# yukara-ikemiya/world-class

Measured on AMD Instinct MI355X. Metric: analysis+synthesis frames/sec (whole node), 48 kHz 5 ms hop, higher is better.
Workload: dtype f64; 1 GPU; 64 synthetic 48 kHz 10 s utterances per GPU (8 distinct, tiled), 5 ms hop, Harvest->CheapTrick->D4C->Synthesis, inputs resident in HBM when the clock starts (`value`; SURVEY.md section 8(d)'s headline with H2D of x and D2H of all outputs inside the clock is `value_with_transfers`); utterances_per_gpu=64, frames_per_gpu=128064, fs=48000, fft_size=2048, parallelism=utterance-sharded x1 (shard.partition), final RCCL all-gather of F0 + checksums

## Files before the change

### world_class_amd/csrc/wc_d4c.hip

```cpp
#include <cmath>
#include <cstdio>
#include <cstdlib>
#include <cstring>
#include <type_traits>
#include <vector>

#include "wc_device.hpp"
#include "wc_internal.hpp"
#include "wc_frames.hpp"
#include "wc_wavefft.hpp"
#include "wc_hostcopy.hpp"

namespace wc {

constexpr double kSafe = 0.000000000001;
constexpr int kMaxBands = 5;

struct D4cArgs {
	const double *x;
	const UttDesc *utts;
	int n_utt;
	const double *tpos, *f0;
	const unsigned long long *rng_off;
	const uint32_t *rng_table;
	unsigned long long rng_base;
	const double2 *tw;
	double *ap;
	double *ap0;
	double *sgd;
	double *coarse;
	uint32_t *cnt;
	const double *nuttall;
	long long total_frames;
	int fs, fft_size_out, n_ap, window_length;
	int select64;
	double threshold;
	long long sgd_stride;
	int *long_list, *long_cnt;
	const int *uidx;
	int rare_only;
	int *rare_list;
	int *lt_list;
	unsigned int *band_tails;
};

template <int N, int T>
__device__ __forceinline__ int d4c_windowed(const double *__restrict__ x, int x_len, int fs, double f0, double pos,
											int type, double ratio, const uint32_t *__restrict__ rng,
											unsigned long long roff, double (&wave)[N / T], double *red, int tid) {
	constexpr int EPT = N / T;
	asm volatile("" : "+v"(tid));
	const int hw = mround(ratio * fs / f0 / 2.0);
	const int wl = 2 * hw + 1;
	const int origin = mround(pos * fs + 0.001);
	const double c1 = 2.0 / ratio / fs;
	double cs0, sn0, csd, snd;
	sincospi(f0 * (c1 * (tid - hw)), &sn0, &cs0);
	sincospi(f0 * (c1 * T), &snd, &csd);
	snd = uniform_d(snd);
	csd = uniform_d(csd);
	auto win = [&](double c) { return type == 1 ? fma(0.5, c, 0.5) : fma(c, fma(0.16, c, 0.5), 0.34); };
	double s1 = 0.0, s2 = 0.0;
	{
		double c = cs0, sn = sn0;
#pragma unroll
		for (int e = 0; e < EPT; ++e) {
			const int i = tid + e * T;
			const bool in = i < wl;
			const double w = in ? win(c) : 0.0;
			const int si = clampi(origin + i - hw, 0, x_len - 1);
			const double noise = randn_at(rng, roff + (in ? i : 0)) * kSafe;
			wave[e] = in ? fma(x[si], w, noise) : 0.0;
			s1 += wave[e];
			s2 += w;
			const double cn = fma(c, csd, -(sn * snd));
			sn = fma(sn, csd, c * snd);
			c = cn;
		}
	}
	block_sum2<T>(s1, s2, red, tid);
	const double wc = uniform_d(s1 / s2);
	{
		double c = cs0, sn = sn0;
#pragma unroll
		for (int e = 0; e < EPT; ++e) {
			const int i = tid + e * T;
			wave[e] = fma(-(i < wl ? win(c) : 0.0), wc, wave[e]);
			const double cn = fma(c, csd, -(sn * snd));
			sn = fma(sn, csd, c * snd);
			c = cn;
		}
// ... 526 lines not shown
		acc = __shfl(acc, first, 64);
		d = __shfl(d, first, 64);
		in_bucket = __shfl(cnt, first, 64);
		need -= acc;
		pre |= ((unsigned long long)d) << shift;
		if (in_bucket == 1u) break;
	}
	double low = 0.0, eq = 0.0, tot = 0.0;
#pragma unroll
	for (int e = 0; e < KEYS; ++e) {
		if (e < nkeys) {
			const double pw = key[e];
			const unsigned long long hb = ((unsigned long long)__double_as_longlong(pw)) >> shift;
			tot += pw;
			low += (hb < (pre >> shift)) ? pw : 0.0;
			eq += (hb == (pre >> shift)) ? pw : 0.0;
		}
	}
	block_sum3<T>(low, eq, tot, red3, tid);
	if (tid == 0) {
		const double thr = (in_bucket == 1u) ? eq : __longlong_as_double((long long)pre);
		const double part = low + (double)need * thr;
		const double cv = 10 * log10(part / tot);
		a.coarse[g * kMaxBands + bnd] = fmin(0.0, cv + (f0 - 100) / 50.0);
	}
}

__global__ __launch_bounds__(256) void d4c_rows_kernel(D4cArgs a) {
	const long long g = blockIdx.x;
	const double f0v = a.f0[g];
	if (f0v == 0.0 || a.ap0[g] <= a.threshold) return;
	const int n_ap = a.n_ap, fs = a.fs;
	const int bins_out = a.fft_size_out / 2 + 1;
	const double *__restrict__ co = a.coarse + g * kMaxBands;
	double *__restrict__ row = a.ap + g * (long long)bins_out;
	const int na = n_ap + 2;
	auto val = [&](int q) { return q == 0 ? -60.0 : (q == na - 1 ? -kSafe : co[q - 1]); };
	for (int k = threadIdx.x; k < bins_out; k += 256) {
		double f = (double)k * fs / a.fft_size_out;
		int c = 1;
		while (c < na && f >= ((c == na - 1) ? fs / 2.0 : c * 3000.0)) ++c;
		c = min(c, na - 1);
		double x0 = (c - 1) * 3000.0;
		double x1 = (c == na - 1) ? fs / 2.0 : c * 3000.0;
		double s = (f - x0) / (x1 - x0);
		double v = val(c - 1) + s * (val(c) - val(c - 1));
		row[k] = exp(v * 0.11512925464970228);
	}
}


constexpr long long kD4Row = 4160;
constexpr int kD4Lds = 2304;

template <int SLOTS>
__device__ __forceinline__ int d4c2_windowed(int type, const double *__restrict__ x, int x_last, int fs, double f0, double pos, double ratio,
											 const uint32_t *__restrict__ rng, int odd, bool weighted, double (&re)[16],
											 double (&im)[16], double &sumsq, int lane) {
	WC_FRESH(lane);
	const int hw = __builtin_amdgcn_readfirstlane(mround(ratio * fs / f0 / 2.0));
	const int wl = 2 * hw + 1;
	const int base = __builtin_amdgcn_readfirstlane(mround(pos * fs + 0.001)) - hw;
	const double c1 = 2.0 / ratio / fs;
	double ce0, se0, co0, so0, cd, sd;
	wf_sincospi(f0 * (c1 * (2 * lane - hw)), se0, ce0);
	wf_sincospi(f0 * (c1 * (2 * lane + 1 - hw)), so0, co0);
	wf_sincospi(f0 * (c1 * 128.0), sd, cd);
	sd = uniform_d(sd);
	cd = uniform_d(cd);
	const double a0 = type == 1 ? 0.5 : 0.34, a2 = type == 1 ? 0.0 : 0.16;
	auto win = [&](double c) { return fma(c, fma(a2, c, 0.5), a0); };
	auto walk = [&](auto loads_c, auto &&body) {
		constexpr int LOADS = decltype(loads_c)::value;
		double ce = ce0, se = se0, co = co0, so = so0;
#pragma unroll
		for (int qg = 0; qg < SLOTS; qg += 4) {
			if (qg * 128 >= wl) break;
			double xs[8];
			uint32_t ns[8];
			const bool ld = LOADS == 1 || (LOADS == 2 && qg >= 16);
			if (ld) {
#pragma unroll
				for (int k = 0; k < 8; ++k) {
					const int i = 2 * lane + 128 * (qg + (k >> 1)) + (k & 1);
					xs[k] = x[clampi(base + i, 0, x_last)];
					ns[k] = rng[i < wl ? i : 0];
				}
				WF_SCHED_FENCE();
			}
#pragma unroll
			for (int k = 0; k < 4; ++k) {
				const int q = qg + k, i0 = 2 * lane + 128 * q;
				const double We = (i0 < wl) ? win(ce) : 0.0, Wo = (i0 + 1 < wl) ? win(co) : 0.0;
				const double ve = (ld && i0 < wl) ? fma(xs[2 * k], We, (ns[2 * k] / 268435456.0 - 6.0) * kSafe) : 0.0;
				const double vo = (ld && i0 + 1 < wl) ? fma(xs[2 * k + 1], Wo, (ns[2 * k + 1] / 268435456.0 - 6.0) * kSafe) : 0.0;
				body(q, i0, We, Wo, ve, vo);
				const double cen = fma(ce, cd, -(se * sd)), con = fma(co, cd, -(so * sd));
				se = fma(se, cd, ce * sd);
				so = fma(so, cd, co * sd);
				ce = cen;
				co = con;
			}
		}
	};
#pragma unroll
	for (int q = 0; q < 16; ++q) re[q] = im[q] = 0.0;
	double s1 = 0.0, s2 = 0.0;
	walk(std::integral_constant<int, 1>(), [&](int q, int, double We, double Wo, double ve, double vo) {
		if (q < 16) { re[q] = ve; im[q] = vo; }
		s1 += ve + vo;
		s2 += We + Wo;
	});
	s1 = wave_sum_all(s1);
	s2 = wave_sum_all(s2);
	const double wc = s1 / s2;
	sumsq = 0.0;
	walk(std::integral_constant<int, 2>(), [&](int q, int i0, double We, double Wo, double ve, double vo) {
		if (q < 16) { ve = re[q]; vo = im[q]; }
		ve = fma(-We, wc, ve);
		vo = fma(-Wo, wc, vo);
		sumsq = fma(vo, vo, fma(ve, ve, sumsq));
		if (weighted) { ve *= i0 + 1.0; vo *= i0 + 2.0; }
		if (q < 16) { re[q] = ve; im[q] = vo; }
		else if (odd) { re[q & 15] -= ve; im[q & 15] -= vo; }
		else { re[q & 15] += ve; im[q & 15] += vo; }
	});
	sumsq = wave_sum_all(sumsq);
	return wl;
}
__device__ __forceinline__ int d4c2_groups(int wl) { return wl > 2048 ? 4 : (wl + 511) >> 9; }

#ifndef WC_D4C2_LT_OCC
#define WC_D4C2_LT_OCC 2
#endif
template <bool LONG>
__device__ __forceinline__ void d4c2_lovetrain_frame(const D4cArgs &a, long long g, double *L, int lane) {
	constexpr int N = 4096, M = 2048;
	const int bins_out = a.fft_size_out / 2 + 1;
	double *__restrict__ row = a.ap + g * (long long)bins_out;
	const double f0v = a.f0[g];
	const int fs = a.fs;
	const double f0c = uniform_d(fmax(f0v, 40.0));
	const bool is_long = f0v != 0.0 && 2 * mround(3.0 * fs / f0c / 2.0) + 1 > 2048;
	if (is_long != LONG) return;
	double ap0 = 0.0;
	if (f0v != 0.0) {
		const int u = a.uidx[g];
		const UttDesc ud = a.utts[u];
		const int b0 = (int)ceil(100.0 * N / fs);
		const int b1 = (int)ceil(4000.0 * N / fs);
		const int b2 = min((int)ceil(7900.0 * N / fs), M);
		double p1 = 0.0, p2 = 0.0;
		double mr[16], mi[16], unused;
		int wl = 0;
		if (!LONG) wl = d4c2_windowed<16>(2, a.x + ud.x_off, ud.x_len - 1, fs, f0c, a.tpos[g], 3.0, a.rng_table + (a.rng_off[g] - a.rng_base), 0,
										  false, mr, mi, unused, lane);
#pragma unroll 1
		for (int odd = 0; odd < 2; ++odd) {
			double re[16], im[16], nyq;
			if (LONG) {
				wl = d4c2_windowed<32>(2, a.x + ud.x_off, ud.x_len - 1, fs, f0c, a.tpos[g], 3.0, a.rng_table + (a.rng_off[g] - a.rng_base), odd,
									   false, re, im, unused, lane);
			} else {
#pragma unroll
				for (int q = 0; q < 16; ++q) { re[q] = mr[q]; im[q] = mi[q]; }
			}
			wf_r2c4096_half(re, im, nyq, d4c2_groups(wl), L, a.tw, lane, odd);
#pragma unroll
			for (int gq = 0; gq < 4; ++gq) {
				const int j = wf_j(lane, odd, gq);
#pragma unroll
				for (int q = 0; q < 4; ++q) {
					const int k = 2 * (j + 256 * q) + odd;
					const double p = fma(re[4 * gq + q], re[4 * gq + q], im[4 * gq + q] * im[4 * gq + q]);
					p2 += (k > b0 && k <= b2) ? p : 0.0;
					p1 += (k > b0 && k <= min(b1, b2)) ? p : 0.0;
				}
			}
// ... 75 lines not shown
			for (int q = 0; q < 4; ++q) L[jg[p][gq] + 512 * q + b] = s.v[p][4 * gq + q] * fs / N;
	if (lane == 0) L[M + b] = s.vM * fs / N;
	{
		const int ke = 2 * lane, ko = 2 * lane + 1;
		if (ke >= 1 && ke <= b) {
			L[b - ke] = s.v[0][0] * fs / N;
			L[M + b + ke] = s.v[0][7] * fs / N;
		}
		if (ko <= b) {
			L[b - ko] = s.v[1][0] * fs / N;
			L[M + b + ko] = s.v[1][7] * fs / N;
		}
	}
	wf_fence();
	if (NONNEG) {
		seq_cumsum_nonneg_wave<36>(L, len, lane);
	} else {
		seq_cumsum_signed_wave<36>(L, len, lane);
	}
	const double step = (double)fs / N;
	const double origin_axis = -(b - 0.5) * fs / N;
	const double rstep = 1.0 / step;
	const double rwidth = uniform_d(1.0 / width);
	auto at = [&](int k) {
		const double lo_axis = (double)k / N * fs - width / 2.0, hi_axis = lo_axis + width;
		return (wf_interp1q(origin_axis, step, rstep, L, len, hi_axis) - wf_interp1q(origin_axis, step, rstep, L, len, lo_axis)) * rwidth;
	};
#pragma unroll
	for (int p = 0; p < 2; ++p)
#pragma unroll
		for (int gq = 0; gq < 4; ++gq) {
#pragma unroll
			for (int q = 0; q < 4; ++q) s.v[p][4 * gq + q] = at(jg[p][gq] + 512 * q);
			WF_SCHED_FENCE();
		}
	s.vM = at(M);
	wf_fence();
}

#ifndef WC_D4C2_OCC
#define WC_D4C2_OCC 2
#endif
#ifndef WC_D4C2_MASTER_LDS
#define WC_D4C2_MASTER_LDS 1
#endif
#ifndef WC_D4C2_TRACE
#define WC_D4C2_TRACE 0
#endif
#if WC_D4C2_TRACE
#define D4_STAMP(i) do { if (lane == 0) reinterpret_cast<unsigned long long *>(park + 4128)[i] = __builtin_readcyclecounter(); } while (0)
#else
#define D4_STAMP(i) do { } while (0)
#endif
#ifndef WC_D4C2_BUFFER
#define WC_D4C2_BUFFER 1
#endif
#if WC_D4C2_BUFFER
typedef unsigned int d4_u2 __attribute__((ext_vector_type(2)));
struct D4Row { __amdgpu_buffer_rsrc_t r; };
__device__ __forceinline__ D4Row d4_row(double *p) {
	D4Row w;
	w.r = __builtin_amdgcn_make_buffer_rsrc(p, 0, (int)(kD4Row * 8), 0x00020000);
	return w;
}
__device__ __forceinline__ double d4_ld(const D4Row &w, int idx) {
	const d4_u2 v = __builtin_amdgcn_raw_buffer_load_b64(w.r, idx * 8, 0, 0);
	return __hiloint2double((int)v.y, (int)v.x);
}
__device__ __forceinline__ void d4_st(const D4Row &w, int idx, double d) {
	d4_u2 v;
	v.x = (unsigned)__double2loint(d);
	v.y = (unsigned)__double2hiint(d);
	__builtin_amdgcn_raw_buffer_store_b64(v, w.r, idx * 8, 0, 0);
}
#else
struct D4Row { double *p; };
__device__ __forceinline__ D4Row d4_row(double *p) { D4Row w; w.p = p; asm volatile("" : "+s"(w.p)); return w; }
__device__ __forceinline__ double d4_ld(const D4Row &w, int idx) { return w.p[idx]; }
__device__ __forceinline__ void d4_st(const D4Row &w, int idx, double d) { w.p[idx] = d; }
#endif
template <bool LONG>
__device__ __forceinline__ void d4c2_frame(const D4cArgs &a, const long long g, double *L, const int lane) {
	constexpr int M = 2048;
	const double f0v = a.f0[g];
	if (f0v == 0.0 || a.ap0[g] <= a.threshold) return;
	const int fs = a.fs;
	const double f0 = uniform_d(fmax(47.0, f0v));
	if (!d4c2_can(f0, fs)) {
		if (!LONG && lane == 0) a.rare_list[1 + atomicAdd(a.rare_list, 1)] = (int)g;
		return;
	}
	const int wl = __builtin_amdgcn_readfirstlane(2 * mround(4.0 * fs / f0 / 2.0) + 1);
	if constexpr (!LONG) {
		if (wl > 2048) {
			if (lane == 0) a.long_list[1 + atomicAdd(a.long_cnt, 1)] = (int)g;
			return;
		}
	}
	const int u = a.uidx[g];
	const UttDesc ud = a.utts[u];
	const double *__restrict__ x = a.x + ud.x_off;
	const int x_last = ud.x_len - 1;
	const double pos = uniform_d(a.tpos[g]);
	const uint32_t *__restrict__ rng = a.rng_table + (a.rng_off[g] - a.rng_base);
#ifdef WC_D4C2_PARK_ALIAS
	double *park = a.sgd + (g & 2047) * a.sgd_stride;
#else
	double *park = a.sgd + g * a.sgd_stride;
#endif
	const D4Row row = d4_row(park);
	D4_STAMP(0);

	const int ng = d4c2_groups(wl);
	double cenM = 0.0, spsM = 0.0;
	if constexpr (!LONG) {
#pragma unroll 1
		for (int job = 0; job < 3; ++job) {
			int ln = lane;
			WC_FRESH(ln);
			const double p = (job == 0) ? pos - 0.25 / f0 : (job == 1) ? pos + 0.25 / f0 : pos;
			double pw;
			{
				double mr[16], mi[16], sumsq;
				d4c2_windowed<16>(job == 2 ? 1 : 2, x, x_last, fs, f0, p, 4.0, rng + (long long)job * wl, 0, false, mr, mi, sumsq, ln);
				pw = (job == 2) ? 1.0 : 0.5 * (1.0 / sqrt(sumsq));
#pragma unroll
				for (int q = 0; q < 16; ++q) {
					if (q < 4 * ng) {
						if (WC_D4C2_MASTER_LDS && job != 2) L[kWfLds + 64 * q + ln] = mr[q] * pw;
						else d4_st(row, 2048 + 64 * q + ln, mr[q] * pw);
						d4_st(row, 3072 + 64 * q + ln, mi[q] * pw);
					}
				}
				if (job == 0) D4_STAMP(1);
			}
			auto master = [&](double (&re)[16], double (&im)[16], bool weighted) {
// ... 12 lines not shown
				if (weighted) {
#pragma unroll
					for (int q = 0; q < 16; ++q) {
						const int i0 = 2 * ln + 128 * q;
						re[q] *= i0 + 1.0;
						im[q] *= i0 + 2.0;
					}
				}
			};
#pragma unroll 1
			for (int odd = 0; odd < 2; ++odd) {
				double re[16], im[16], nyq1;
				master(re, im, false);
				wf_r2c4096_half(re, im, nyq1, ng, L, a.tw, ln, odd);
				if (job == 0 && odd == 0) D4_STAMP(2);
				if (job == 2) {
					double pwr[16];
#pragma unroll
					for (int s = 0; s < 16; ++s) pwr[s] = 0.25 * fma(re[s], re[s], im[s] * im[s]);
					if (odd == 0) {
						spsM = 0.25 * (nyq1 * nyq1);
#pragma unroll
						for (int s = 0; s < 16; ++s) L[kWfLds + 64 * s + ln] = pwr[s];
					} else {
#pragma unroll
						for (int s = 0; s < 16; ++s) {
							d4_st(row, 3072 + 64 * s + ln, pwr[s]);
							d4_st(row, 2048 + 64 * s + ln, L[kWfLds + 64 * s + ln]);
						}
					}
				} else {
					double ar[16], ai[16], nyq2;
					master(ar, ai, true);
					wf_r2c4096_half(ar, ai, nyq2, ng, L, a.tw, ln, odd);
					double acc[16];
#pragma unroll
					for (int s = 0; s < 16; ++s) acc[s] = fma(re[s], ar[s], im[s] * ai[s]);
					if (job == 1) {
						double prev[16];
#pragma unroll
						for (int s = 0; s < 16; ++s) prev[s] = d4_ld(row, 1024 * odd + 64 * s + ln);
						WF_SCHED_FENCE();
#pragma unroll
						for (int s = 0; s < 16; ++s) acc[s] += prev[s];
					}
#pragma unroll
					for (int s = 0; s < 16; ++s) d4_st(row, 1024 * odd + 64 * s + ln, acc[s]);
					if (odd == 0) cenM += nyq1 * nyq2;
					if (job == 0 && odd == 0) D4_STAMP(3);
				}
			}
			if (job == 0) D4_STAMP(4);
		}
	} else
#pragma unroll 1
	for (int odd = 0; odd < 2; ++odd) {
		double acc[16], accM = 0.0;
#pragma unroll
		for (int s = 0; s < 16; ++s) acc[s] = 0.0;
#pragma unroll 1
		for (int job = 0; job < 3; ++job) {
			int ln = lane;
			WC_FRESH(ln);
			double ar[16], ai[16], re[16], im[16], sumsq, nyq1;
			const double p = (job == 0) ? pos - 0.25 / f0 : (job == 1) ? pos + 0.25 / f0 : pos;
			d4c2_windowed<32>(job == 2 ? 1 : 2, x, x_last, fs, f0, p, 4.0, rng + (long long)job * wl, odd, false, ar, ai, sumsq, ln);
			if (odd == 0 && job == 0) D4_STAMP(1);
			const double pw = (job == 2) ? 1.0 : 0.5 * (1.0 / sqrt(sumsq));
#pragma unroll
			for (int q = 0; q < 16; ++q) {
				re[q] = ar[q] * pw;
				im[q] = ai[q] * pw;
			}
			wf_r2c4096_half(re, im, nyq1, ng, L, a.tw, lane, odd);
			if (odd == 0 && job == 0) D4_STAMP(2);
			if (job == 2) {
#pragma unroll
				for (int s = 0; s < 16; ++s) d4_st(row, 2048 + 1024 * odd + 64 * s + ln, 0.25 * fma(re[s], re[s], im[s] * im[s]));
				if (odd == 0) spsM = 0.25 * (nyq1 * nyq1);
			} else {
				double nyq2;
				if (wl > 2048) {
					d4c2_windowed<32>(2, x, x_last, fs, f0, p, 4.0, rng + (long long)job * wl, odd, true, ar, ai, sumsq, ln);
#pragma unroll
					for (int q = 0; q < 16; ++q) { ar[q] *= pw; ai[q] *= pw; }
				} else {
#pragma unroll
					for (int q = 0; q < 16; ++q) {
						const int i0 = 2 * ln + 128 * q;
						ar[q] *= pw * (i0 + 1.0);
						ai[q] *= pw * (i0 + 2.0);
					}
				}
				wf_r2c4096_half(ar, ai, nyq2, ng, L, a.tw, lane, odd);
#pragma unroll
				for (int s = 0; s < 16; ++s) acc[s] += fma(re[s], ar[s], im[s] * ai[s]);
				accM += nyq1 * nyq2;
				if (odd == 0 && job == 0) D4_STAMP(3);
			}
		}
#pragma unroll
		for (int s = 0; s < 16; ++s) d4_st(row, 1024 * odd + 64 * s + lane, acc[s]);
		if (odd == 0) cenM = accM;
		if (odd == 0) D4_STAMP(4);
	}
	D4_STAMP(5);
	D4Bins cen, sps;
#pragma unroll
	for (int p = 0; p < 2; ++p)
#pragma unroll
		for (int s = 0; s < 16; ++s) {
			cen.v[p][s] = d4_ld(row, 1024 * p + 64 * s + lane);
			sps.v[p][s] = d4_ld(row, 2048 + 1024 * p + 64 * s + lane);
		}
	cen.vM = cenM;
	sps.vM = spsM;
	D4_STAMP(6);
	d4c2_dc_correction(cen, f0, fs, L, lane);
	d4c2_dc_correction(sps, f0, fs, L, lane);
	D4_STAMP(7);
	d4c2_smooth<true>(sps, f0, fs, L, lane);
	D4_STAMP(8);
#pragma unroll
	for (int p = 0; p < 2; ++p)
#pragma unroll
		for (int s = 0; s < 16; ++s) cen.v[p][s] = cen.v[p][s] / sps.v[p][s];
	cen.vM = cen.vM / sps.vM;
#pragma unroll 1
	for (int it = 0; it < 2; ++it) {
		d4c2_smooth<false>(cen, it ? f0 : f0 / 2.0, fs, L, lane);
		if (it == 0) sps = cen;
	}
	D4_STAMP(9);
#pragma unroll
	for (int p = 0; p < 2; ++p)
#pragma unroll
		for (int gq = 0; gq < 4; ++gq) {
			const int j = 2 * wf_j(lane, p, gq) + p;
#pragma unroll
			for (int q = 0; q < 4; ++q) d4_st(row, j + 512 * q, sps.v[p][4 * gq + q] - cen.v[p][4 * gq + q]);
		}
	if (lane == 0) d4_st(row, M, sps.vM - cen.vM);
	D4_STAMP(10);
}

template <bool LONG>
__global__ __launch_bounds__(64) __attribute__((amdgpu_waves_per_eu(WC_D4C2_OCC, WC_D4C2_OCC))) void d4c2_frames_kernel(D4cArgs a) {
	__shared__ __attribute__((aligned(16))) double L[kD4Lds];
	const int lane = threadIdx.x;
	if constexpr (!LONG) {
		const long long g = xcd_frame(blockIdx.x, a.total_frames);
		if (g >= a.total_frames) return;
		d4c2_frame<false>(a, g, L, lane);
	} else {
		const int n_long = *a.long_cnt;
#pragma unroll 1
		for (int i = blockIdx.x; i < n_long; i += gridDim.x) {
			d4c2_frame<true>(a, a.long_list[1 + i], L, lane);
			wf_fence();
		}
	}
}

#ifndef WC_D4C2_BAND_OCC
#define WC_D4C2_BAND_OCC 2
#endif
#ifndef WC_D4C2_BRACKET
#define WC_D4C2_BRACKET 1
#endif
#ifndef WC_D4C2_BRACKET_FIRST
#define WC_D4C2_BRACKET_FIRST 0x1p-14
#endif
#ifndef WC_D4C2_BAND_PF
#define WC_D4C2_BAND_PF 0
#endif
template <int WAVES>
__global__ __launch_bounds__(64) __attribute__((amdgpu_waves_per_eu(WAVES == 3 ? 3 : WC_D4C2_BAND_OCC, WAVES == 3 ? 3 : WC_D4C2_BAND_OCC))) void d4c2_band_kernel(D4cArgs a) {
	constexpr int N = 4096, M = 2048;
	constexpr bool W3 = WAVES == 3;
	__shared__ __attribute__((aligned(16))) double L[kWfLds + (W3 ? kWfT2Lds : 0)];
	const double *T2 = W3 ? L + kWfLds : nullptr;
	if constexpr (W3) __builtin_assume(T2 != nullptr);
	const int lane = threadIdx.x;
	const int n_ap = a.n_ap;
	const long long blk = xcd_frame(blockIdx.x, (long long)gridDim.x);
	const long long g = blk / n_ap;
	const int bnd = (int)(blk % n_ap);
	if (g >= a.total_frames) return;
	const double f0v = a.f0[g];
	if (f0v == 0.0 || a.ap0[g] <= a.threshold) return;
	if constexpr (W3) wf_t2_to_lds(L + kWfLds, a.tw, lane);
	const double f0 = fmax(47.0, f0v);
	const int fs = a.fs;
	const int wln = a.window_length, hwl = wln / 2;
	const int boundary = mround(N * 8.0 / wln);
	const unsigned int K = (unsigned int)(M + 1 - boundary - 1);
	const int center = (int)(3000.0 * (bnd + 1) * N / fs);
	const double *__restrict__ src = a.sgd + g * a.sgd_stride + (center - hwl);
	const int ng = wln > 512 ? 2 : 1;
	double key[2][16], keyM = 0.0;
	[[maybe_unused]] double pf = 0.0;
	auto half = [&](auto parity) {
		constexpr int odd = decltype(parity)::value;
		double re[16], im[16], nyq;
		int ln = lane;
		if constexpr (W3) WC_FRESH(ln);
		{
			double sv[16], nv[16];
#pragma unroll
			for (int k = 0; k < 16; ++k) {
				const int i = min(2 * ln + 128 * (k >> 1) + (k & 1), wln - 1);
				sv[k] = src[i];
				nv[k] = a.nuttall[i];
// ... 459 lines not shown
		while (hi_h - lo_h > 1 && c_lo != K) {
			const int mid = lo_h + ((hi_h - lo_h) >> 1);
			const unsigned int c = count_hi(mid);
			if (c >= K) hi_h = mid;
			if (c <= K) { lo_h = mid; c_lo = c; }
		}
		lo = lo_h < 0 ? -1ll : (((long long)lo_h << 32) | 0xFFFFFFFFll);
		hi = min(hi, ((long long)hi_h << 32) | 0xFFFFFFFFll);
	} else {
#pragma unroll 1
		for (int tr = 0; tr < 2; ++tr) {
			const long long cand = __double_as_longlong(mx * (tr == 0 ? WC_D4C2_BRACKET_FIRST : 0x1p-40));
			const unsigned int c = count_le(cand);
			if (c <= K && cand > 0) { lo = cand; c_lo = c; break; }
			hi = cand > 0 && c >= K ? cand : hi;
		}
	}
	for (int it = 0; it < 64 && hi - lo > 1 && c_lo != K; ++it) {
		const long long mid = lo + ((hi - lo) >> 1);
		const unsigned int c = count_le(mid);
		if (c >= K) hi = mid;
		if (c <= K) { lo = mid; c_lo = c; }
		if (c == K) break;
	}
	double low = 0.0, tot = 0.0;
#pragma unroll
	for (int s = 0; s < 16; ++s) {
		tot += key[s];
		low += (__double_as_longlong(key[s]) <= lo) ? key[s] : 0.0;
	}
	if (lane == 0) {
		tot += keyM;
		low += (__double_as_longlong(keyM) <= lo) ? keyM : 0.0;
	}
	low = wave_sum_all(low);
	tot = wave_sum_all(tot);
	if (lane == 0) {
		const double part = low + (double)(K - c_lo) * __longlong_as_double(hi);
		const double cv = 10 * log10(part / tot);
		a.coarse[g * kMaxBands + bnd] = fmin(0.0, cv + (f0 - 100) / 50.0);
	}
}

}

using namespace wc;

struct wc_d4c {
	int fs, fft_size_d4c, fft_size_lt, n_ap, window_length;
	double threshold;
	bool select64 = false;
	int band_waves = 3;
	bool lt_listed = true;
	bool count_tails = false;
	bool split;
	bool wave2;
	Device *dev;
	double f0_bound = 0.0;
	DevBuf nuttall, utts, cnt, uidx, long_list, rare_list, lt_list, tails, off, endpos, endpos2, ap0, sgd, coarse, d_x, d_tpos, d_f0, d_ap;
	HostBuf h_stage, h_rows, h_x;
};

template <int N>
static void launch_lt(const D4cArgs &a, hipStream_t s) {
	long long blocks = ((a.total_frames + 7) / 8) * 8;
	constexpr int TL = (N >= 8192) ? 1024 : (N / 8 < 64 ? 64 : N / 8);
	hipLaunchKernelGGL((d4c_lovetrain_kernel<N, TL>), dim3((unsigned)blocks), dim3(TL), 0, s, a);
}
template <int N>
static void launch_main(const D4cArgs &a, hipStream_t s, bool split, int part) {
	long long blocks = ((a.total_frames + 7) / 8) * 8;
	constexpr int TF = (N >= 8192) ? 1024 : (N / 8 < 64 ? 64 : N / 8);
	if (part == 0) {
		if (!split) hipLaunchKernelGGL((d4c_frames_kernel<N, TF, false>), dim3((unsigned)blocks), dim3(TF), 0, s, a);
		else hipLaunchKernelGGL((d4c_frames_kernel<N, TF, true>), dim3((unsigned)blocks), dim3(TF), 0, s, a);
		return;
	}
	if (a.n_ap > 0) hipLaunchKernelGGL((d4c_band_kernel<N, TF>), dim3((unsigned)(blocks * a.n_ap)), dim3(TF), 0, s, a);
	hipLaunchKernelGGL(d4c_rows_kernel, dim3((unsigned)a.total_frames), dim3(256), 0, s, a);
}

int d4c_enqueue(wc_d4c *d, hipStream_t s, int n_utt, const double *d_x, const int *x_length, const double *d_tpos,
				const double *d_f0, const int *f0_length, int fft_size, double *d_ap, const uint64_t *rng_pos,
				const unsigned long long *d_start) {
	Device *dev = d->dev;
	if (fft_size < 2 || (fft_size & 1)) return fail(WC_ERR_INVALID, "d4c: fft_size must be even and positive");
	std::vector<UttDesc> utts(n_utt);
	long long xo = 0, fo = 0;
	uint64_t min_pos = ~0ull, max_end = 0;
	const uint64_t lt_max = (uint64_t)(2 * (int)(3.0 * d->fs / 40.0 / 2.0 + 1.0) + 1);
	const uint64_t main_max = 3ull * (uint64_t)(2 * (int)(4.0 * d->fs / 47.0 / 2.0 + 1.0) + 1);
	for (int u = 0; u < n_utt; ++u) {
		if (x_length[u] <= 0 || f0_length[u] < 0) return fail(WC_ERR_INVALID, "d4c: non-positive length");
		UttDesc &t = utts[u];
		t.x_off = xo; t.f_off = fo; t.y_off = 0;
		t.x_len = x_length[u]; t.f_len = f0_length[u]; t.y_len = 0; t.f_base = 0;
		t.rng_pos = rng_pos ? rng_pos[u] : 0ull;
		xo += x_length[u];
		fo += f0_length[u];
		if (t.rng_pos < min_pos) min_pos = t.rng_pos;
		uint64_t e = t.rng_pos + (lt_max + main_max) * (uint64_t)t.f_len;
		if (e > max_end) max_end = e;
	}
	const long long total = fo;
	(void)min_pos; (void)max_end;
	if (total == 0) return WC_OK;
	int rc;
	if ((rc = d->utts.reserve(sizeof(UttDesc) * n_utt))) return rc;
	if ((rc = d->cnt.reserve(sizeof(uint32_t) * total))) return rc;
	if ((rc = d->uidx.reserve(sizeof(int) * total))) return rc;
	if ((rc = d->long_list.reserve(sizeof(int) * (total + 1)))) return rc;
	if ((rc = d->rare_list.reserve(sizeof(int) * (total + 1)))) return rc;
	if ((rc = d->off.reserve(sizeof(uint64_t) * total))) return rc;
	if ((rc = d->ap0.reserve(sizeof(double) * total))) return rc;
	const bool split = d->split;
	const bool main2 = d->wave2 && split && (d->fft_size_d4c == 4096 || d->fft_size_d4c == 2048) && d->window_length <= 1023;
	const long long row2 = d->fft_size_d4c == 4096 ? kD4Row : kD4Row1;
	if (split) {
		if ((rc = d->sgd.reserve(sizeof(double) * (size_t)total * (main2 ? (size_t)row2 : (size_t)(d->fft_size_d4c / 2 + 1))))) return rc;
		if ((rc = d->coarse.reserve(sizeof(double) * (size_t)total * kMaxBands))) return rc;
	}
	if ((rc = d->endpos.reserve(sizeof(uint64_t) * n_utt))) return rc;
	if ((rc = d->endpos2.reserve(sizeof(uint64_t) * n_utt))) return rc;
	if ((rc = d->h_stage.reserve(sizeof(UttDesc) * n_utt + sizeof(uint64_t) * n_utt))) return rc;
	std::memcpy(d->h_stage.p, utts.data(), sizeof(UttDesc) * n_utt);
	WC_HIP(hipMemcpyAsync(d->utts.p, d->h_stage.p, sizeof(UttDesc) * n_utt, hipMemcpyHostToDevice, s));
	if ((rc = d->h_stage.mark(s))) return rc;
	const unsigned grid1 = (unsigned)((total + 255) / 256);
	const bool lt_listed = d->lt_listed && d->wave2 && d->fft_size_lt == 4096;
	if (lt_listed) {
		if ((rc = d->lt_list.reserve(sizeof(int) * (total + 1)))) return rc;
		WC_HIP(hipMemsetAsync(d->lt_list.p, 0, sizeof(int), s));
	}
	if (d->count_tails) {
		if ((rc = d->tails.reserve(sizeof(unsigned int)))) return rc;
		WC_HIP(hipMemsetAsync(d->tails.p, 0, sizeof(unsigned int), s));
	}
	hipLaunchKernelGGL(d4c_lt_count_kernel, dim3(grid1), dim3(256), 0, s, d_f0, total, d->fs, d->cnt.as<uint32_t>(), d->utts.as<UttDesc>(), n_utt,
					   d->uidx.as<int>(), d->long_list.as<int>(), d->rare_list.as<int>(), lt_listed ? d->lt_list.as<int>() : nullptr);
	hipLaunchKernelGGL(utt_scan_kernel, dim3(n_utt), dim3(256), 0, s, d->cnt.as<uint32_t>(), d->utts.as<UttDesc>(),
					   d_start, d->off.as<unsigned long long>(), d->endpos.as<unsigned long long>());
	D4cArgs a;
	a.x = d_x; a.utts = d->utts.as<UttDesc>(); a.n_utt = n_utt; a.tpos = d_tpos; a.f0 = d_f0;
	a.rng_off = d->off.as<unsigned long long>(); a.rng_table = dev->rng_table.as<uint32_t>(); a.rng_base = dev->rng_base;
	a.tw = dev->twiddle; a.ap = d_ap; a.ap0 = d->ap0.as<double>(); a.cnt = d->cnt.as<uint32_t>(); a.uidx = d->uidx.as<int>(); a.long_cnt = d->long_list.as<int>(); a.long_list = d->long_list.as<int>();
	a.sgd = d->sgd.as<double>(); a.coarse = d->coarse.as<double>();
	a.nuttall = d->nuttall.as<double>(); a.total_frames = total; a.fs = d->fs; a.fft_size_out = fft_size;
	a.n_ap = d->n_ap; a.window_length = d->window_length; a.threshold = d->threshold; a.select64 = d->select64 ? 1 : 0;
	a.rare_only = 0;
	a.rare_list = d->rare_list.as<int>();
	a.lt_list = lt_listed ? d->lt_list.as<int>() : nullptr;
	a.band_tails = d->count_tails ? d->tails.as<unsigned int>() : nullptr;
	a.sgd_stride = main2 ? row2 : (long long)(d->fft_size_d4c / 2 + 1);
	const long long blocks8 = ((total + 7) / 8) * 8;
	if ((rc = dev->time_begin("d4c_lovetrain", s))) return rc;
	if (d->wave2 && d->fft_size_lt == 4096) {
		hipLaunchKernelGGL(d4c2_lovetrain_kernel<false>, dim3((unsigned)blocks8), dim3(64), 0, s, a);
		hipLaunchKernelGGL(d4c2_lovetrain_kernel<true>, dim3((unsigned)(lt_listed ? std::min<long long>(blocks8, 4096) : blocks8)), dim3(64), 0, s, a);
	} else if (d->wave2 && d->fft_size_lt == 2048) {
		hipLaunchKernelGGL(d4c1_lovetrain_kernel, dim3((unsigned)blocks8), dim3(64), 0, s, a);
	}
	else switch (d->fft_size_lt) {
		case 1024: launch_lt<1024>(a, s); break;
		case 2048: launch_lt<2048>(a, s); break;
		case 4096: launch_lt<4096>(a, s); break;
		case 8192: launch_lt<8192>(a, s); break;
		default: return fail(WC_ERR_UNSUPPORTED, "d4c: unsupported LoveTrain FFT size (fs must be 8..96 kHz)");
	}
	WC_HIP(hipGetLastError());
	if ((rc = dev->time_end("d4c_lovetrain", s))) return rc;
	hipLaunchKernelGGL(utt_scan_kernel, dim3(n_utt), dim3(256), 0, s, d->cnt.as<uint32_t>(), d->utts.as<UttDesc>(),
					   d->endpos.as<unsigned long long>(), d->off.as<unsigned long long>(), d->endpos2.as<unsigned long long>());
	for (int part = 0; part < (split ? 2 : 1); ++part) {
		const char *name = part == 0 ? "d4c_frames" : "d4c_bands";
		if ((rc = dev->time_begin(name, s))) return rc;
		if (main2 && part == 0) {
			a.rare_only = 1;
			if (d->fft_size_d4c == 4096) {
				hipLaunchKernelGGL(d4c2_frames_kernel<false>, dim3((unsigned)blocks8), dim3(64), 0, s, a);
				hipLaunchKernelGGL(d4c2_frames_kernel<true>, dim3((unsigned)std::min<long long>(blocks8, 4096)), dim3(64), 0, s, a);
				hipLaunchKernelGGL((d4c_frames_kernel<4096, 512, true, true>), dim3(256), dim3(512), 0, s, a);
			} else {
				hipLaunchKernelGGL(d4c1_frames_kernel, dim3((unsigned)blocks8), dim3(64), 0, s, a);
				hipLaunchKernelGGL((d4c_frames_kernel<2048, 256, true, true>), dim3(256), dim3(256), 0, s, a);
			}
			a.rare_only = 0;
		} else if (main2 && part == 1) {
			if (a.n_ap > 0) {
				if (d->fft_size_d4c == 4096 && d->band_waves == 3 && !d->select64) hipLaunchKernelGGL(d4c2_band_kernel<3>, dim3((unsigned)(blocks8 * a.n_ap)), dim3(64), 0, s, a);
				else if (d->fft_size_d4c == 4096) hipLaunchKernelGGL(d4c2_band_kernel<2>, dim3((unsigned)(blocks8 * a.n_ap)), dim3(64), 0, s, a);
				else hipLaunchKernelGGL(d4c1_band_kernel, dim3((unsigned)(blocks8 * a.n_ap)), dim3(64), 0, s, a);
			}
			hipLaunchKernelGGL(d4c_rows_kernel, dim3((unsigned)a.total_frames), dim3(256), 0, s, a);
		} else
		switch (d->fft_size_d4c) {
			case 1024: launch_main<1024>(a, s, split, part); break;
			case 2048: launch_main<2048>(a, s, split, part); break;
			case 4096: launch_main<4096>(a, s, split, part); break;
			case 8192: launch_main<8192>(a, s, split, part); break;
			default: return fail(WC_ERR_UNSUPPORTED, "d4c: unsupported FFT size (fs must be 8..96 kHz)");
		}
		WC_HIP(hipGetLastError());
		if ((rc = dev->time_end(name, s))) return rc;
	}
#if WC_D4C2_TRACE
	if (const char *path = getenv("WC_D4C_TRACE")) {
		std::vector<double> row((size_t)kD4Row);
		std::vector<unsigned long long> out;
		WC_HIP(hipStreamSynchronize(s));
		for (long long g = 0; g < total; g += 7) {
			WC_HIP(hipMemcpy(row.data(), d->sgd.as<double>() + g * kD4Row, sizeof(double) * kD4Row, hipMemcpyDeviceToHost));
			const unsigned long long *st = reinterpret_cast<const unsigned long long *>(row.data() + 4128);
			out.insert(out.end(), st, st + 16);
		}
		if (FILE *f = fopen(path, "wb")) { fwrite(out.data(), 8, out.size(), f); fclose(f); }
	}
#endif
	return WC_OK;
}

extern "C" int wc_debug_d4c_band_tails(wc_d4c *d, unsigned int *tails) {
	if (!d || !tails || !d->count_tails || !d->tails.p) return fail(WC_ERR_INVALID, "d4c: no tail count on this handle");
	WC_HIP(hipSetDevice(d->dev->id));
	DeviceLock lock(d->dev);
	WC_HIP(hipStreamSynchronize(d->dev->active()));
	WC_HIP(hipMemcpy(tails, d->tails.p, sizeof(unsigned int), hipMemcpyDeviceToHost));
	return WC_OK;
}

extern "C" int wc_debug_d4c_lt_listed(wc_d4c *d, int *n) {
	if (!d || !n) return fail(WC_ERR_INVALID, "d4c: null argument");
	*n = -1;
	if (!(d->lt_listed && d->wave2 && d->fft_size_lt == 4096) || !d->lt_list.p) return WC_OK;
	WC_HIP(hipSetDevice(d->dev->id));
	DeviceLock lock(d->dev);
	WC_HIP(hipStreamSynchronize(d->dev->active()));
	WC_HIP(hipMemcpy(n, d->lt_list.p, sizeof(int), hipMemcpyDeviceToHost));
	return WC_OK;
}

extern "C" int wc_debug_d4c_bands(wc_d4c *d, int n_frames, const double *rows, double *coarse) {
	if (!d || n_frames <= 0 || !rows || !coarse) return fail(WC_ERR_INVALID, "d4c: null argument");
	if (d->fft_size_d4c != 4096 || d->window_length > 1023 || d->n_ap <= 0) return fail(WC_ERR_UNSUPPORTED, "d4c: no 4096-point band stage at this rate");
	constexpr long long row = 2049;
	WC_HIP(hipSetDevice(d->dev->id));
	DeviceLock lock(d->dev);
	hipStream_t s = d->dev->active();
	int rc;
	const long long blocks8 = ((n_frames + 7) / 8) * 8;
	if ((rc = d->sgd.reserve(sizeof(double) * (size_t)(n_frames * row)))) return rc;
	if ((rc = d->coarse.reserve(sizeof(double) * (size_t)n_frames * kMaxBands))) return rc;
	if ((rc = d->d_f0.reserve(sizeof(double) * (size_t)n_frames))) return rc;
	if ((rc = d->ap0.reserve(sizeof(double) * (size_t)n_frames))) return rc;
	std::vector<double> f0((size_t)n_frames, 100.0), ap0((size_t)n_frames, 2.0);
	WC_HIP(hipMemcpy(d->sgd.p, rows, sizeof(double) * (size_t)(n_frames * row), hipMemcpyHostToDevice));
	WC_HIP(hipMemcpy(d->d_f0.p, f0.data(), sizeof(double) * (size_t)n_frames, hipMemcpyHostToDevice));
	WC_HIP(hipMemcpy(d->ap0.p, ap0.data(), sizeof(double) * (size_t)n_frames, hipMemcpyHostToDevice));
	WC_HIP(hipMemsetAsync(d->coarse.p, 0, sizeof(double) * (size_t)n_frames * kMaxBands, s));
	if (d->count_tails) {
		if ((rc = d->tails.reserve(sizeof(unsigned int)))) return rc;
		WC_HIP(hipMemsetAsync(d->tails.p, 0, sizeof(unsigned int), s));
	}
	D4cArgs a = {};
	a.f0 = d->d_f0.as<double>(); a.ap0 = d->ap0.as<double>(); a.threshold = 1.0; a.tw = d->dev->twiddle;
	a.sgd = d->sgd.as<double>(); a.sgd_stride = row; a.coarse = d->coarse.as<double>(); a.nuttall = d->nuttall.as<double>();
	a.total_frames = n_frames; a.fs = d->fs; a.n_ap = d->n_ap; a.window_length = d->window_length; a.select64 = d->select64 ? 1 : 0;
	a.band_tails = d->count_tails ? d->tails.as<unsigned int>() : nullptr;
	if (d->band_waves == 3 && !d->select64) hipLaunchKernelGGL(d4c2_band_kernel<3>, dim3((unsigned)(blocks8 * a.n_ap)), dim3(64), 0, s, a);
	else hipLaunchKernelGGL(d4c2_band_kernel<2>, dim3((unsigned)(blocks8 * a.n_ap)), dim3(64), 0, s, a);
	WC_HIP(hipGetLastError());
	WC_HIP(hipStreamSynchronize(s));
	WC_HIP(hipMemcpy(coarse, d->coarse.p, sizeof(double) * (size_t)n_frames * kMaxBands, hipMemcpyDeviceToHost));
	return WC_OK;
}

void d4c_set_f0_bound(wc_d4c *d, double f0_bound) { d->f0_bound = f0_bound; }
const unsigned long long *d4c_end_positions(const wc_d4c *d) { return d->endpos2.as<unsigned long long>(); }

uint64_t d4c_draw_bound(const wc_d4c *d, int f0_length) {
	const uint64_t lt_max = (uint64_t)(2 * (int)(3.0 * d->fs / 40.0 / 2.0 + 1.0) + 1);
	const uint64_t main_max = 3ull * (uint64_t)(2 * (int)(4.0 * d->fs / 47.0 / 2.0 + 1.0) + 1);
	return (lt_max + main_max) * (uint64_t)(f0_length > 0 ? f0_length : 0);
}

static int d4c_run_device(wc_d4c *d, int n_utt, const double *d_x, const int *x_length, const double *d_tpos,
						  const double *d_f0, const int *f0_length, int fft_size, double *d_ap, uint64_t *rng_pos) {
	Device *dev = d->dev;
	hipStream_t s = dev->active();
	int rc;
	uint64_t lo = ~0ull, hi = 0;
	long long total = 0;
	for (int u = 0; u < n_utt; ++u) {
		uint64_t p0 = rng_pos ? rng_pos[u] : 0ull;
		lo = p0 < lo ? p0 : lo;
		uint64_t e = p0 + d4c_draw_bound(d, f0_length[u]);
		hi = e > hi ? e : hi;
		total += f0_length[u] > 0 ? f0_length[u] : 0;
	}
	if ((rc = dev->ensure_rng(lo, hi))) return rc;
	if ((rc = d4c_enqueue(d, s, n_utt, d_x, x_length, d_tpos, d_f0, f0_length, fft_size, d_ap, rng_pos, nullptr))) return rc;
	if (rng_pos && total > 0) {
		std::vector<uint64_t> h_end(n_utt);
		WC_HIP(hipMemcpyAsync(h_end.data(), d->endpos2.p, sizeof(uint64_t) * n_utt, hipMemcpyDeviceToHost, s));
		WC_HIP(hipStreamSynchronize(s));
		for (int u = 0; u < n_utt; ++u) rng_pos[u] = h_end[u];
	}
	return WC_OK;
}

wc::Device *d4c_device(const wc_d4c *d) { return d->dev; }

extern "C" {

wc_d4c *wc_d4c_create(int fs, double threshold) {
	if (fs <= 0) { set_error("d4c: fs must be positive"); return nullptr; }
	Device *dev = current_device();
	if (!dev) return nullptr;
	wc_d4c *d = new wc_d4c();
	d->fs = fs;
	d->threshold = threshold;
	d->dev = dev;
	{
		const char *sp = getenv("WC_D4C_SPLIT");
		d->split = !(sp && sp[0] == '0');
		const char *sel = getenv("WC_D4C_SELECT");
		d->select64 = sel && std::strcmp(sel, "64") == 0;
		const char *bw = getenv("WC_D4C_BAND_WAVES");
		if (bw && (std::strcmp(bw, "2") == 0 || std::strcmp(bw, "3") == 0)) d->band_waves = bw[0] - '0';
		const char *ll = getenv("WC_D4C_LT_LIST");
		d->lt_listed = !(ll && ll[0] == '0');
		const char *ct = getenv("WC_D4C_BAND_TAILS");
		d->count_tails = ct && ct[0] == '1';
		const char *impl = getenv("WC_D4C_IMPL");
		d->wave2 = !(impl && std::strcmp(impl, "block") == 0);
	}
	d->fft_size_d4c = static_cast<int>(std::pow(2.0, 1.0 + static_cast<int>(std::log(4.0 * fs / 47.0 + 1) / 0.69314718055994529)));
	d->n_ap = static_cast<int>(std::fmin(15000.0, fs / 2.0 - 3000.0) / 3000.0);
	d->window_length = static_cast<int>(3000.0 * d->fft_size_d4c / fs) * 2 + 1;
	d->fft_size_lt = static_cast<int>(std::pow(2.0, 1.0 + static_cast<int>(std::log(3.0 * fs / 40.0 + 1) / 0.69314718055994529)));
	if (d->n_ap < 0) d->n_ap = 0;
	if (d->n_ap > kMaxBands || (d->fft_size_d4c != 1024 && d->fft_size_d4c != 2048 && d->fft_size_d4c != 4096 && d->fft_size_d4c != 8192) ||
		(d->fft_size_lt != 1024 && d->fft_size_lt != 2048 && d->fft_size_lt != 4096 && d->fft_size_lt != 8192)) {
		set_error("d4c: unsupported sampling rate (supported: 8 kHz .. 96 kHz)");
		delete d;
		return nullptr;
	}
	std::vector<double> win(d->window_length);
	for (int i = 0; i < d->window_length; ++i) {
		double t = i / (d->window_length - 1.0);
		win[i] = 0.355768 - 0.487396 * std::cos(2.0 * 3.1415926535897932384 * t) +
				 0.144232 * std::cos(4.0 * 3.1415926535897932384 * t) - 0.012604 * std::cos(6.0 * 3.1415926535897932384 * t);
	}
	if (d->nuttall.reserve(sizeof(double) * win.size()) ||
		hipMemcpy(d->nuttall.p, win.data(), sizeof(double) * win.size(), hipMemcpyHostToDevice) != hipSuccess) {
		set_error("d4c: window upload failed");
		delete d;
		return nullptr;
	}
	dev->handle_born();
	return d;
}
void wc_d4c_destroy(wc_d4c *d) {
	if (!d) return;
	d->dev->quiesce();
	d->dev->handle_gone();
	d->nuttall.release(); d->utts.release(); d->cnt.release(); d->uidx.release(); d->long_list.release(); d->rare_list.release(); d->lt_list.release(); d->tails.release(); d->off.release(); d->endpos.release(); d->endpos2.release();
	d->ap0.release(); d->sgd.release(); d->coarse.release(); d->d_x.release(); d->d_tpos.release(); d->d_f0.release(); d->d_ap.release(); d->h_stage.release(); d->h_rows.release(); d->h_x.release();
	delete d;
}

int wc_d4c_compute_device(wc_d4c *d, int n_utt, const double *d_x, const int *x_length, const double *d_tpos,
						  const double *d_f0, const int *f0_length, int fft_size, double *d_ap, uint64_t *rng_pos) {
	if (!d || n_utt <= 0 || !d_x || !x_length || !d_tpos || !d_f0 || !f0_length || !d_ap)
		return fail(WC_ERR_INVALID, "d4c: null argument");
	WC_HIP(hipSetDevice(d->dev->id));
	DeviceLock lock(d->dev);
	return d4c_run_device(d, n_utt, d_x, x_length, d_tpos, d_f0, f0_length, fft_size, d_ap, rng_pos);
}

int wc_d4c_compute(wc_d4c *d, const double *x, int x_length, const double *temporal_positions, const double *f0,
				   int f0_length, int fft_size, double **aperiodicity) {
	if (!d || !x || !temporal_positions || !f0 || !aperiodicity) return fail(WC_ERR_INVALID, "d4c: null argument");
	if (x_length <= 0 || f0_length < 0) return fail(WC_ERR_INVALID, "d4c: bad length");
	if (f0_length == 0) return WC_OK;
	WC_HIP(hipSetDevice(d->dev->id));
	DeviceLock lock(d->dev);
	hipStream_t s = d->dev->active();
	const int bins = fft_size / 2 + 1;
	int rc;
	if ((rc = d->d_x.reserve(sizeof(double) * x_length))) return rc;
	if ((rc = d->d_tpos.reserve(sizeof(double) * f0_length))) return rc;
	if ((rc = d->d_f0.reserve(sizeof(double) * f0_length))) return rc;
	if ((rc = d->d_ap.reserve(sizeof(double) * (size_t)f0_length * bins))) return rc;
	if ((rc = array_up(s, x, (size_t)x_length, d->h_x, d->d_x.as<double>()))) return rc;
	WC_HIP(hipMemcpyAsync(d->d_tpos.p, temporal_positions, sizeof(double) * f0_length, hipMemcpyHostToDevice, s));
	WC_HIP(hipMemcpyAsync(d->d_f0.p, f0, sizeof(double) * f0_length, hipMemcpyHostToDevice, s));
	uint64_t pos = global_rng_position();
	rc = d4c_run_device(d, 1, d->d_x.as<double>(), &x_length, d->d_tpos.as<double>(), d->d_f0.as<double>(), &f0_length,
						fft_size, d->d_ap.as<double>(), &pos);
	if (rc) return rc;
	set_global_rng_position(pos);
	const size_t n_ap = (size_t)f0_length * bins;
	if ((rc = d->h_rows.reserve(sizeof(double) * n_ap))) return rc;
	return rows_down(s, aperiodicity, f0_length, bins, d->d_ap.as<double>(), d->h_rows.as<double>());
}

}
```

Before: 5.211 million frames/s.

## Park long-window D4C waveforms in global scratch instead of recomputing per half

Adds a parked path for long-window D4C frames: the windowed waveform is computed once per job and written to a per-block global scratch buffer, then reloaded for each odd/even FFT half and for the weighted variant. Previously the long path regenerated the windowed signal (sincos, rng, window) several times per job. This trades recomputation for extra global-memory traffic and a scratch allocation, and the old behaviour stays available through WC_D4C_LONG=halves. Only frames with windows longer than 2048 samples take this path.

```diff
diff --git a/world_class_amd/csrc/wc_d4c.hip b/world_class_amd/csrc/wc_d4c.hip
--- a/world_class_amd/csrc/wc_d4c.hip
+++ b/world_class_amd/csrc/wc_d4c.hip
@@ -37,6 +37,7 @@
 	double threshold;
 	long long sgd_stride;
 	int *long_list, *long_cnt;
+	double *long_park;
 	const int *uidx;
 	int rare_only;
 	int *rare_list;
@@ -669,11 +670,17 @@
 
 constexpr long long kD4Row = 4160;
 constexpr int kD4Lds = 2304;
-
-template <int SLOTS>
+constexpr long long kD4Park = 4096;
+constexpr long long kD4LongGrid = 4096;
+
+struct D4NoPark {
+	__device__ __forceinline__ void operator()(int, double, double) const {}
+};
+template <int SLOTS, class Park = D4NoPark>
 __device__ __forceinline__ int d4c2_windowed(int type, const double *__restrict__ x, int x_last, int fs, double f0, double pos, double ratio,
 											 const uint32_t *__restrict__ rng, int odd, bool weighted, double (&re)[16],
-											 double (&im)[16], double &sumsq, int lane) {
+											 double (&im)[16], double &sumsq, int lane, Park park = Park()) {
+	constexpr bool PARKED = !std::is_same<Park, D4NoPark>::value;
 	WC_FRESH(lane);
 	const int hw = __builtin_amdgcn_readfirstlane(mround(ratio * fs / f0 / 2.0));
 	const int wl = 2 * hw + 1;
@@ -737,10 +744,14 @@
 		ve = fma(-We, wc, ve);
 		vo = fma(-Wo, wc, vo);
 		sumsq = fma(vo, vo, fma(ve, ve, sumsq));
-		if (weighted) { ve *= i0 + 1.0; vo *= i0 + 2.0; }
-		if (q < 16) { re[q] = ve; im[q] = vo; }
-		else if (odd) { re[q & 15] -= ve; im[q & 15] -= vo; }
-		else { re[q & 15] += ve; im[q & 15] += vo; }
+		if constexpr (PARKED) {
+			park(q, ve, vo);
+		} else {
+			if (weighted) { ve *= i0 + 1.0; vo *= i0 + 2.0; }
+			if (q < 16) { re[q] = ve; im[q] = vo; }
+			else if (odd) { re[q & 15] -= ve; im[q & 15] -= vo; }
+			else { re[q & 15] += ve; im[q & 15] += vo; }
+		}
 	});
 	sumsq = wave_sum_all(sumsq);
 	return wl;
@@ -922,15 +933,16 @@
 #else
 #define D4_STAMP(i) do { } while (0)
 #endif
+constexpr int kD4Short = 0, kD4Long = 1, kD4LongHalves = 2;
 #ifndef WC_D4C2_BUFFER
 #define WC_D4C2_BUFFER 1
 #endif
 #if WC_D4C2_BUFFER
 typedef unsigned int d4_u2 __attribute__((ext_vector_type(2)));
 struct D4Row { __amdgpu_buffer_rsrc_t r; };
-__device__ __forceinline__ D4Row d4_row(double *p) {
+__device__ __forceinline__ D4Row d4_row(double *p, long long n = kD4Row) {
 	D4Row w;
-	w.r = __builtin_amdgcn_make_buffer_rsrc(p, 0, (int)(kD4Row * 8), 0x00020000);
+	w.r = __builtin_amdgcn_make_buffer_rsrc(p, 0, (int)(n * 8), 0x00020000);
 	return w;
 }
 __device__ __forceinline__ double d4_ld(const D4Row &w, int idx) {
@@ -945,13 +957,14 @@
 }
 #else
 struct D4Row { double *p; };
-__device__ __forceinline__ D4Row d4_row(double *p) { D4Row w; w.p = p; asm volatile("" : "+s"(w.p)); return w; }
+__device__ __forceinline__ D4Row d4_row(double *p, long long = kD4Row) { D4Row w; w.p = p; asm volatile("" : "+s"(w.p)); return w; }
 __device__ __forceinline__ double d4_ld(const D4Row &w, int idx) { return w.p[idx]; }
 __device__ __forceinline__ void d4_st(const D4Row &w, int idx, double d) { w.p[idx] = d; }
 #endif
-template <bool LONG>
+template <int FORM>
 __device__ __forceinline__ void d4c2_frame(const D4cArgs &a, const long long g, double *L, const int lane) {
 	constexpr int M = 2048;
+	constexpr bool LONG = FORM != kD4Short;
 	const double f0v = a.f0[g];
 	if (f0v == 0.0 || a.ap0[g] <= a.threshold) return;
 	const int fs = a.fs;
@@ -1070,6 +1083,104 @@
 			}
 			if (job == 0) D4_STAMP(4);
 		}
+	} else if constexpr (FORM == kD4Long) {
+		const D4Row win = d4_row(a.long_park + (long long)blockIdx.x * kD4Park, kD4Park);
+#pragma unroll 1
+		for (int job = 0; job < 3; ++job) {
+			int ln = lane;
+			WC_FRESH(ln);
+			const double p = (job == 0) ? pos - 0.25 / f0 : (job == 1) ? pos + 0.25 / f0 : pos;
+			double pw;
+			{
+				double mr[16], mi[16], sumsq;
+				d4c2_windowed<32>(job == 2 ? 1 : 2, x, x_last, fs, f0, p, 4.0, rng + (long long)job * wl, 0, false, mr, mi, sumsq, ln,
+								  [&](int q, double ve, double vo) {
+									  d4_st(win, 64 * q + ln, ve);
+									  d4_st(win, 2048 + 64 * q + ln, vo);
+								  });
+				pw = (job == 2) ? 1.0 : 0.5 * (1.0 / sqrt(sumsq));
+				if (job == 0) D4_STAMP(1);
+			}
+			auto master = [&](double (&re)[16], double (&im)[16], bool weighted, int odd) {
+				int ln = lane;
+				WC_FRESH(ln);
+#pragma unroll
+				for (int q = 0; q < 16; ++q) {
+					re[q] = d4_ld(win, 64 * q + ln);
+					im[q] = d4_ld(win, 2048 + 64 * q + ln);
+				}
+				WF_SCHED_FENCE();
+				if (weighted) {
+#pragma unroll
+					for (int q = 0; q < 16; ++q) {
+						const int i0 = 2 * ln + 128 * q;
+						re[q] *= i0 + 1.0;
+						im[q] *= i0 + 2.0;
+					}
+				}
+#pragma unroll
+				for (int qg = 16; qg < 32; qg += 8) {
+					if (qg * 128 >= wl) break;
+					const bool two = (qg + 4) * 128 < wl;
+					double ur[8], ui[8];
+#pragma unroll
+					for (int k = 0; k < 8; ++k) {
+						ur[k] = ui[k] = 0.0;
+						if (k < 4 || two) {
+							ur[k] = d4_ld(win, 64 * (qg + k) + ln);
+							ui[k] = d4_ld(win, 2048 + 64 * (qg + k) + ln);
+						}
+					}
+					WF_SCHED_FENCE();
+#pragma unroll
+					for (int k = 0; k < 8; ++k) {
+						if (k < 4 || two) {
+							const int q = qg + k, i0 = 2 * ln + 128 * q;
+							double ve = ur[k], vo = ui[k];
+							if (weighted) { ve *= i0 + 1.0; vo *= i0 + 2.0; }
+							if (odd) { re[q & 15] -= ve; im[q & 15] -= vo; }
+							else { re[q & 15] += ve; im[q & 15] += vo; }
+						}
+					}
+				}
+#pragma unroll
+				for (int q = 0; q < 16; ++q) {
+					re[q] *= pw;
+					im[q] *= pw;
+				}
+			};
+#pragma unroll 1
+			for (int odd = 0; odd < 2; ++odd) {
+				double re[16], im[16], nyq1;
+				master(re, im, false, odd);
+				wf_r2c4096_half(re, im, nyq1, 4, L, a.tw, ln, odd);
+				if (job == 0 && odd == 0) D4_STAMP(2);
+				if (job == 2) {
+#pragma unroll
+					for (int s = 0; s < 16; ++s) d4_st(row, 2048 + 1024 * odd + 64 * s + ln, 0.25 * fma(re[s], re[s], im[s] * im[s]));
+					if (odd == 0) spsM = 0.25 * (nyq1 * nyq1);
+				} else {
+					double ar[16], ai[16], nyq2;
+					master(ar, ai, true, odd);
+					wf_r2c4096_half(ar, ai, nyq2, 4, L, a.tw, ln, odd);
+					double acc[16];
+#pragma unroll
+					for (int s = 0; s < 16; ++s) acc[s] = 0.0;
+					if (job == 1) {
+#pragma unroll
+						for (int s = 0; s < 16; ++s) acc[s] = d4_ld(row, 1024 * odd + 64 * s + ln);
+						WF_SCHED_FENCE();
+					}
+#pragma unroll
+					for (int s = 0; s < 16; ++s) acc[s] += fma(re[s], ar[s], im[s] * ai[s]);
+#pragma unroll
+					for (int s = 0; s < 16; ++s) d4_st(row, 1024 * odd + 64 * s + ln, acc[s]);
+					if (odd == 0) cenM += nyq1 * nyq2;
+					if (job == 0 && odd == 0) D4_STAMP(3);
+				}
+			}
+			if (job == 0) D4_STAMP(4);
+		}
 	} else
 #pragma unroll 1
 	for (int odd = 0; odd < 2; ++odd) {
@@ -1169,14 +1280,24 @@
 	if constexpr (!LONG) {
 		const long long g = xcd_frame(blockIdx.x, a.total_frames);
 		if (g >= a.total_frames) return;
-		d4c2_frame<false>(a, g, L, lane);
+		d4c2_frame<kD4Short>(a, g, L, lane);
 	} else {
 		const int n_long = *a.long_cnt;
 #pragma unroll 1
 		for (int i = blockIdx.x; i < n_long; i += gridDim.x) {
-			d4c2_frame<true>(a, a.long_list[1 + i], L, lane);
+			d4c2_frame<kD4Long>(a, a.long_list[1 + i], L, lane);
 			wf_fence();
 		}
+	}
+}
+__global__ __launch_bounds__(64) __attribute__((amdgpu_waves_per_eu(WC_D4C2_OCC, WC_D4C2_OCC))) void d4c2_frames_halves_kernel(D4cArgs a) {
+	__shared__ __attribute__((aligned(16))) double L[kD4Lds];
+	const int lane = threadIdx.x;
+	const int n_long = *a.long_cnt;
+#pragma unroll 1
+	for (int i = blockIdx.x; i < n_long; i += gridDim.x) {
+		d4c2_frame<kD4LongHalves>(a, a.long_list[1 + i], L, lane);
+		wf_fence();
 	}
 }
 
@@ -1742,12 +1863,13 @@
 	bool select64 = false;
 	int band_waves = 3;
 	bool lt_listed = true;
+	bool long_halves = false;
 	bool count_tails = false;
 	bool split;
 	bool wave2;
 	Device *dev;
 	double f0_bound = 0.0;
-	DevBuf nuttall, utts, cnt, uidx, long_list, rare_list, lt_list, tails, off, endpos, endpos2, ap0, sgd, coarse, d_x, d_tpos, d_f0, d_ap;
+	DevBuf nuttall, utts, cnt, uidx, long_list, long_park, rare_list, lt_list, tails, off, endpos, endpos2, ap0, sgd, coarse, d_x, d_tpos, d_f0, d_ap;
 	HostBuf h_stage, h_rows, h_x;
 };
 
@@ -1810,6 +1932,9 @@
 		if ((rc = d->sgd.reserve(sizeof(double) * (size_t)total * (main2 ? (size_t)row2 : (size_t)(d->fft_size_d4c / 2 + 1))))) return rc;
 		if ((rc = d->coarse.reserve(sizeof(double) * (size_t)total * kMaxBands))) return rc;
 	}
+	const long long long_grid = std::min<long long>(((total + 7) / 8) * 8, kD4LongGrid);
+	const bool long_parked = main2 && d->fft_size_d4c == 4096 && !d->long_halves;
+	if (long_parked && (rc = d->long_park.reserve(sizeof(double) * (size_t)(long_grid * kD4Park)))) return rc;
 	if ((rc = d->endpos.reserve(sizeof(uint64_t) * n_utt))) return rc;
 	if ((rc = d->endpos2.reserve(sizeof(uint64_t) * n_utt))) return rc;
 	if ((rc = d->h_stage.reserve(sizeof(UttDesc) * n_utt + sizeof(uint64_t) * n_utt))) return rc;
@@ -1834,7 +1959,7 @@
 	a.x = d_x; a.utts = d->utts.as<UttDesc>(); a.n_utt = n_utt; a.tpos = d_tpos; a.f0 = d_f0;
 	a.rng_off = d->off.as<unsigned long long>(); a.rng_table = dev->rng_table.as<uint32_t>(); a.rng_base = dev->rng_base;
 	a.tw = dev->twiddle; a.ap = d_ap; a.ap0 = d->ap0.as<double>(); a.cnt = d->cnt.as<uint32_t>(); a.uidx = d->uidx.as<int>(); a.long_cnt = d->long_list.as<int>(); a.long_list = d->long_list.as<int>();
-	a.sgd = d->sgd.as<double>(); a.coarse = d->coarse.as<double>();
+	a.sgd = d->sgd.as<double>(); a.coarse = d->coarse.as<double>(); a.long_park = long_parked ? d->long_park.as<double>() : nullptr;
 	a.nuttall = d->nuttall.as<double>(); a.total_frames = total; a.fs = d->fs; a.fft_size_out = fft_size;
 	a.n_ap = d->n_ap; a.window_length = d->window_length; a.threshold = d->threshold; a.select64 = d->select64 ? 1 : 0;
 	a.rare_only = 0;
@@ -1868,7 +1993,8 @@
 			a.rare_only = 1;
 			if (d->fft_size_d4c == 4096) {
 				hipLaunchKernelGGL(d4c2_frames_kernel<false>, dim3((unsigned)blocks8), dim3(64), 0, s, a);
-				hipLaunchKernelGGL(d4c2_frames_kernel<true>, dim3((unsigned)std::min<long long>(blocks8, 4096)), dim3(64), 0, s, a);
+				if (long_parked) hipLaunchKernelGGL(d4c2_frames_kernel<true>, dim3((unsigned)long_grid), dim3(64), 0, s, a);
+				else hipLaunchKernelGGL(d4c2_frames_halves_kernel, dim3((unsigned)long_grid), dim3(64), 0, s, a);
 				hipLaunchKernelGGL((d4c_frames_kernel<4096, 512, true, true>), dim3(256), dim3(512), 0, s, a);
 			} else {
 				hipLaunchKernelGGL(d4c1_frames_kernel, dim3((unsigned)blocks8), dim3(64), 0, s, a);
@@ -1915,6 +2041,17 @@
 	DeviceLock lock(d->dev);
 	WC_HIP(hipStreamSynchronize(d->dev->active()));
 	WC_HIP(hipMemcpy(tails, d->tails.p, sizeof(unsigned int), hipMemcpyDeviceToHost));
+	return WC_OK;
+}
+
+extern "C" int wc_debug_d4c_long_count(wc_d4c *d, int *n) {
+	if (!d || !n) return fail(WC_ERR_INVALID, "d4c: null argument");
+	*n = -1;
+	if (!(d->wave2 && d->split && d->fft_size_d4c == 4096 && d->window_length <= 1023) || !d->long_list.p) return WC_OK;
+	WC_HIP(hipSetDevice(d->dev->id));
+	DeviceLock lock(d->dev);
+	WC_HIP(hipStreamSynchronize(d->dev->active()));
+	WC_HIP(hipMemcpy(n, d->long_list.p, sizeof(int), hipMemcpyDeviceToHost));
 	return WC_OK;
 }
 
@@ -2019,6 +2156,8 @@
 		if (bw && (std::strcmp(bw, "2") == 0 || std::strcmp(bw, "3") == 0)) d->band_waves = bw[0] - '0';
 		const char *ll = getenv("WC_D4C_LT_LIST");
 		d->lt_listed = !(ll && ll[0] == '0');
+		const char *lw = getenv("WC_D4C_LONG");
+		d->long_halves = lw && std::strcmp(lw, "halves") == 0;
 		const char *ct = getenv("WC_D4C_BAND_TAILS");
 		d->count_tails = ct && ct[0] == '1';
 		const char *impl = getenv("WC_D4C_IMPL");
@@ -2054,7 +2193,7 @@
 	if (!d) return;
 	d->dev->quiesce();
 	d->dev->handle_gone();
-	d->nuttall.release(); d->utts.release(); d->cnt.release(); d->uidx.release(); d->long_list.release(); d->rare_list.release(); d->lt_list.release(); d->tails.release(); d->off.release(); d->endpos.release(); d->endpos2.release();
+	d->nuttall.release(); d->utts.release(); d->cnt.release(); d->uidx.release(); d->long_list.release(); d->long_park.release(); d->rare_list.release(); d->lt_list.release(); d->tails.release(); d->off.release(); d->endpos.release(); d->endpos2.release();
 	d->ap0.release(); d->sgd.release(); d->coarse.release(); d->d_x.release(); d->d_tpos.release(); d->d_f0.release(); d->d_ap.release(); d->h_stage.release(); d->h_rows.release(); d->h_x.release();
 	delete d;
 }
```

Result: faster. 5.269 million frames/s, median of 6 (+1.1%).
